# neyuru/RayTracing

Hardware: AMD Instinct MI355X
Metric: ray-steps/sec (whole node) on vert_heterogeneous, 1M rays; % HBM roofline (higher is better)
Workload: dtype f64

## Files before the change

### include/rtmi.h

```cpp
#ifndef RTMI_H
#define RTMI_H

#include <stdint.h>

#ifdef __cplusplus
extern "C" {
#endif

#define RTMI_ABI_VERSION 7

typedef enum {
    RTMI_OK = 0,
    RTMI_ERR_ARG = -1,
    RTMI_ERR_HIP = -2,
    RTMI_ERR_ALLOC = -3,
    RTMI_ERR_STATE = -4,
    RTMI_ERR_UNSUPPORTED = -5
} rtmi_status;

typedef enum { RTMI_INTERFACE = 1, RTMI_FISHEYE = 2, RTMI_VERT_HETEROGENEOUS = 3, RTMI_ANISOTROPY = 4 } rtmi_scenario;

typedef enum { RTMI_OP_MIN = 1, RTMI_OP_MAX = 11 } rtmi_method_range;

typedef enum { RTMI_F64 = 0, RTMI_F32 = 1 } rtmi_dtype;
// ... 221 lines not shown
int rtmi_kirchhoff_lsqr(rtmi_kirchhoff *k, const rtmi_lsqr_params *lp, const double *data, double *x, double *history,
                        rtmi_lsqr_stats *st);

typedef struct {
    void *s_ray, *n_ray;
    double *x, *y, *theta;
    void *n, *gx, *gy;
    double *dist_sim, *dist_real, *T;
    int32_t *istep;
    const int32_t *perm;
    int64_t R, rec_rows;
    int32_t dtype, record_stride;
} rtmi_device_view;
int rtmi_batch_view(rtmi_batch *b, rtmi_device_view *v);

#define RTMI_AUTO_SAMPLES 3
typedef struct {
    uint64_t ray_steps;
    uint64_t live_rays;
    double kernel_ms;
    uint32_t launches;
    uint32_t vgprs, sgprs, lds_bytes;
    uint32_t launch_mode_used;
    double kernel_ms_total;
    uint64_t launches_total;
    uint32_t auto_fallbacks;
    uint32_t auto_kept;
    double auto_ms[2][RTMI_AUTO_SAMPLES];
    uint32_t auto_n[2];
    uint32_t retraced;
    uint32_t retrace_overflow;
    uint64_t retraced_total;
    uint32_t dispatch_first;
    uint32_t reserved_;
} rtmi_stats;
int rtmi_batch_stats(rtmi_batch *b, rtmi_stats *s);
void rtmi_batch_destroy(rtmi_batch *b);

typedef struct rtmi_shard rtmi_shard;
typedef enum {
    RTMI_SHARD_AUTO = 0,
    RTMI_SHARD_RCCL = 1,
    RTMI_SHARD_COPY = 2
} rtmi_shard_transport;
int rtmi_shard_create(int scenario, double xi, double xs, double yi, double ys, double delta, const rtmi_params *p, int64_t R,
                      const double *x0, const double *y0, const double *theta0, const int *devices, int ndev, int transport,
                      rtmi_shard **out);
int rtmi_shard_run(rtmi_shard *s);
int rtmi_shard_reset(rtmi_shard *s);
int rtmi_shard_read_d_ray(rtmi_shard *s, double *d_ray);
int rtmi_shard_read_final(rtmi_shard *s, double *final9);
int rtmi_shard_gather_rows(rtmi_shard *s, int64_t row0, int64_t nrows, int64_t every, double **rows_dev);
int rtmi_shard_read_rows(rtmi_shard *s, int64_t row0, int64_t nrows, int64_t every, double *s_ray);
typedef struct {
    int32_t ndev, transport;
    int64_t R;
    uint64_t ray_steps, live_rays;
    double run_seconds;
    double kernel_ms_max;
    uint32_t auto_fallbacks, reserved_;
} rtmi_shard_stats;
int rtmi_shard_info(rtmi_shard *s, rtmi_shard_stats *st);
int rtmi_shard_batch(rtmi_shard *s, int i, rtmi_batch **b, int *device);
void rtmi_shard_destroy(rtmi_shard *s);

int rtmi_debug_sincos(int64_t n, const double *x, double *s, double *c);
int rtmi_debug_arctan2(int64_t n, const double *y, const double *x, double *out);
// ... 23 lines not shown
```

### raytracing_amd/_lib.py

```python
import ctypes as C
import os

_HERE = os.path.dirname(os.path.abspath(__file__))
LIB_PATH = os.environ.get("RTMI_LIB_PATH") or os.path.join(_HERE, "librtmi.so")

ABI_VERSION = 7
AUTO_SAMPLES = 3
LAUNCH_AUTO, LAUNCH_REFILL, LAUNCH_SLICED, LAUNCH_PLAIN = 0, 1, 2, 3
LAUNCH_MODES = {"auto": LAUNCH_AUTO, "refill": LAUNCH_REFILL, "sliced": LAUNCH_SLICED, "plain": LAUNCH_PLAIN, "lane": LAUNCH_PLAIN}
LAUNCH_NAMES = {LAUNCH_AUTO: "auto", LAUNCH_REFILL: "refill", LAUNCH_SLICED: "sliced", LAUNCH_PLAIN: "plain"}

_dp = C.POINTER(C.c_double)
_ip = C.POINTER(C.c_int32)


class RtmiError(RuntimeError):
    def __init__(self, code, msg):
        super().__init__(f"librtmi error {code}: {msg}")
        self.code = code


class Params(C.Structure):
    _fields_ = [("method", C.c_int32), ("dtype", C.c_int32), ("gamma", C.c_double), ("gamma_step", C.c_double),
                ("step", C.c_double), ("max_size", C.c_int32), ("record_stride", C.c_int32), ("rec_rows", C.c_int64),
                ("box", C.c_double * 4), ("launch_mode", C.c_int32), ("block_size", C.c_int32),
                ("refill_min", C.c_int32), ("exact_basis", C.c_int32),
                ("field_path", C.c_int32), ("sort_rays", C.c_int32),
                ("ext_s_ray", C.c_void_p), ("ext_n_ray", C.c_void_p), ("lazy_clear", C.c_int32), ("no_n_ray", C.c_int32), ("slice_steps", C.c_int32),
                ("reference_order", C.c_int32), ("no_retrace", C.c_int32)]


class DeviceView(C.Structure):
    _fields_ = [("s_ray", C.c_void_p), ("n_ray", C.c_void_p), ("x", C.c_void_p), ("y", C.c_void_p),
                ("theta", C.c_void_p), ("n", C.c_void_p), ("gx", C.c_void_p), ("gy", C.c_void_p),
                ("dist_sim", C.c_void_p), ("dist_real", C.c_void_p), ("T", C.c_void_p), ("istep", C.c_void_p),
                ("perm", C.c_void_p),
                ("R", C.c_int64), ("rec_rows", C.c_int64), ("dtype", C.c_int32), ("record_stride", C.c_int32)]


class Stats(C.Structure):
    _fields_ = [("ray_steps", C.c_uint64), ("live_rays", C.c_uint64), ("kernel_ms", C.c_double),
                ("launches", C.c_uint32), ("vgprs", C.c_uint32), ("sgprs", C.c_uint32), ("lds_bytes", C.c_uint32),
                ("launch_mode_used", C.c_uint32), ("kernel_ms_total", C.c_double), ("launches_total", C.c_uint64),
                ("auto_fallbacks", C.c_uint32), ("auto_kept", C.c_uint32),
                ("auto_ms", (C.c_double * AUTO_SAMPLES) * 2), ("auto_n", C.c_uint32 * 2),
                ("retraced", C.c_uint32), ("retrace_overflow", C.c_uint32), ("retraced_total", C.c_uint64),
                ("dispatch_first", C.c_uint32), ("reserved_", C.c_uint32)]


class ShardStats(C.Structure):
    _fields_ = [("ndev", C.c_int32), ("transport", C.c_int32), ("R", C.c_int64), ("ray_steps", C.c_uint64), ("live_rays", C.c_uint64),
                ("run_seconds", C.c_double), ("kernel_ms_max", C.c_double), ("auto_fallbacks", C.c_uint32), ("reserved_", C.c_uint32)]


class TwoPointParams(C.Structure):
    _fields_ = [("max_arrivals", C.c_int32), ("max_crossings", C.c_int32), ("max_iter", C.c_int32), ("reserved0", C.c_int32),
                ("tol", C.c_double), ("mem_budget", C.c_int64), ("reserved", C.c_int64 * 4)]


class TwoPointStats(C.Structure):
    _fields_ = [("iterations", C.c_int32), ("groups", C.c_int32), ("rec_rows", C.c_int64), ("overflow", C.c_uint64),
                ("fan_ms", C.c_double), ("bracket_ms", C.c_double), ("refine_ms", C.c_double), ("reserved", C.c_double * 4)]


class GridParams(C.Structure):
    _fields_ = [("gx0", C.c_double), ("gdx", C.c_double), ("nx", C.c_int64), ("gy0", C.c_double), ("gdy", C.c_double),
                ("ny", C.c_int64), ("max_gap", C.c_double), ("max_dtheta", C.c_double), ("amplitude", C.c_int32),
                ("reserved0", C.c_int32), ("reserved", C.c_int64 * 4)]


class GridStats(C.Structure):
    _fields_ = [("cells", C.c_int64), ("skipped_cells", C.c_int64), ("triangles", C.c_int64), ("folded", C.c_int64),
                ("atomics", C.c_uint64 * 3), ("pass_ms", C.c_double * 3), ("max_gap", C.c_double), ("max_dtheta", C.c_double),
                ("reserved", C.c_double * 4)]


class ArrivalParams(C.Structure):
    _fields_ = [("karr", C.c_int32), ("order", C.c_int32), ("reserved", C.c_int64 * 4)]


# ... 230 lines not shown
```

### raytracing_amd/csrc/rtmi.hip

```cpp
#include <hip/hip_runtime.h>

#include <chrono>
#include <cmath>
#include <cstdio>
#include <cstdlib>
#include <algorithm>
#include <cstring>
#include <exception>
#include <mutex>
#include <numeric>
#include <new>
#include <string>
#include <thread>
#include <utility>
#include <vector>

#include "rt_device.h"
#include "rtmi_field.h"

static thread_local std::string g_err;
static int fail(int code, const std::string& msg) {
    g_err = msg;
    return code;
}
// ... 360 lines not shown
__device__ __forceinline__ void row_store(__amdgpu_buffer_rsrc_t rs, int voff, int soff, double v) {
    __builtin_amdgcn_raw_buffer_store_b64(__builtin_bit_cast(rt_u32x2, v), rs, voff, soff, kRowStoreAux);
}
__device__ __forceinline__ void row_store(__amdgpu_buffer_rsrc_t rs, int voff, int soff, float v) {
    __builtin_amdgcn_raw_buffer_store_b32(__builtin_bit_cast(unsigned, v), rs, voff, soff, kRowStoreAux);
}
template <typename T>
__device__ __forceinline__ T* wave_uniform_ptr(T* p) {
    const unsigned long v = (unsigned long)p;
    const unsigned lo = __builtin_amdgcn_readfirstlane((unsigned)v), hi = __builtin_amdgcn_readfirstlane((unsigned)(v >> 32));
    return (T*)(((unsigned long)hi << 32) | lo);
}
template <typename T>
__device__ __forceinline__ void write_row_uniform(const BatchDev<T>& a, T* rowp, T* nrowp, int voff, const rt::Ray<T>& r) {
    int qR = (int)(a.R * (long)sizeof(T));
    asm volatile("" : "+s"(qR));
    rowp = wave_uniform_ptr(rowp);
    nrowp = wave_uniform_ptr(nrowp);
    const __amdgpu_buffer_rsrc_t rs = __builtin_amdgcn_make_buffer_rsrc(rowp, 0, 0x7fffffff, 0x00020000);
    row_store(rs, voff, 0, (T)r.x);
    row_store(rs, voff, qR, (T)r.y);
    row_store(rs, voff, 2 * qR, r.mx);
    row_store(rs, voff, 3 * qR, r.my);
    row_store(rs, voff, 4 * qR, (T)r.tt);
    row_store(rs, voff, 5 * qR, (T)r.th);
    if (nrowp) {
        const __amdgpu_buffer_rsrc_t rn = __builtin_amdgcn_make_buffer_rsrc(nrowp, 0, 0x7fffffff, 0x00020000);
        row_store(rn, voff, 0, r.nray);
    }
}

template <typename T, int METHOD, bool ISO, typename G, bool UROW, bool COH = false>
__device__ __forceinline__ void advance_loop(const BatchDev<T>& a, const rt::Consts<T>& K, G& gather, rt::Ray<T>& r, long k, int& i,
                                             bool& alive, int max_size, int nsteps, long blk) {
    const bool RECORD = a.stride != 0;
    int stride = a.stride;
    asm volatile("" : "+s"(stride));
    int until = 0;
    long row = 0;
    int rows_left = 0;
    T *rowp = nullptr, *nrowp = nullptr;
    const int voff = (int)(threadIdx.x * sizeof(T));
    if (UROW && RECORD) {
        const int i0 = __builtin_amdgcn_readfirstlane(rt::wave_max_i(alive ? i : 0));
        const int row0 = i0 / stride;
        until = stride - (i0 % stride);
        rows_left = (int)(a.rec_rows - 1 - row0 < 0x7fffffffL ? a.rec_rows - 1 - row0 : 0x7fffffffL);
        rowp = a.s_ray + (size_t)row0 * 6 * a.R + blk;
        nrowp = a.n_ray ? a.n_ray + (size_t)row0 * a.R + blk : nullptr;
    } else if (RECORD && alive) {
        until = stride - (i % stride);
        row = i / stride;
    }
    constexpr bool HOV = rt::ReportsSteep<G>::value && rt::RotatesUnit<T, METHOD>::value;
    auto one_step = [&]() -> bool {
        if (rt_ballot(alive) == 0ull) return false;
        const bool active = alive;
        ++i;
        const bool inside = rt::ray_step<T, METHOD, ISO>(a.F, K, gather, active, r, i);
        if (UROW && RECORD) {
            if (--until == 0) {
                until = stride;
                rowp += 6 * a.R;
                if (nrowp) nrowp += a.R;
                if (--rows_left >= 0 && active) write_row_uniform(a, rowp, nrowp, voff, r);
            }
        }
        if (active) {
            if (!UROW && RECORD) {
                if (--until == 0) {
                    until = stride;
                    ++row;
                    if (row < a.rec_rows) write_row(a, row, k, r);
                }
            }
// ... 2 lines not shown
                if constexpr (rt::IsExact<T, METHOD>::value) rt::ex::finish_state<rt::base_method(METHOD)>(a.F, gather, r);
                const BatchDev<T> ab = rare_batch(a);
                if constexpr (HOV) {
                    if (r.hov == INFINITY) {
                        store_ray<T, METHOD, COH, true>(ab, k, r, i, false);
                        __builtin_amdgcn_s_waitcnt(0x0F70);
                        if (!push_critical(ab, k, i)) {
                            r.hov = -INFINITY;
                            alive = !rt::outside(K, r) && (i + 1 < max_size);
                            if (alive) st_state<COH>(ab.alive + k, (unsigned char)1);
                        }
                        return true;
                    }
                }
                store_ray<T, METHOD, COH, HOV>(ab, k, r, i, false);
            }
        }
        if constexpr (rt::HasPrefetch<G>::value) gather.prefetch(a.F, alive, (T)r.x + r.ux * K.step, (T)r.y + r.uy * K.step);
        return true;
    };
    if constexpr (!rt::IsExact<T, METHOD>::value) {
        for (int it = 0; it < nsteps; it += 2) {
            if (!one_step()) break;
            if (it + 1 >= nsteps) break;
            if (!one_step()) break;
        }
    } else {
        for (int it = 0; it < nsteps; ++it)
            if (!one_step()) break;
    }
}

template <typename T, int METHOD, bool ISO, bool LDS, bool VAR, bool COH = false, bool NOFLAT = false, bool LAT = false, bool LAYER = false>
__device__ __forceinline__ bool advance_bundle(const BatchDev<T>& a, T* lds, long blk, int nsteps);

__device__ __forceinline__ unsigned xcd_grouped_block(unsigned h, unsigned nblocks) {
    constexpr unsigned G = 8;
    constexpr unsigned ROUND = 8u * G;
    if (h < nblocks / ROUND * ROUND) {
        const unsigned xcd = h & 7u, idx = h >> 3;
        return ((idx / G) * 8u + xcd) * G + idx % G;
    }
    return h;
}

constexpr bool light_method(int m) { return m == 2 || m == 6 || m == 1 || m == 7 || m == 8; }
constexpr bool heavy_method(int m) { return m == 4 || m == 5 || m >= 9; }
template <typename T> constexpr int advance_waves(int m, bool lds, int f32_waves) {
    return sizeof(T) == 4 ? f32_waves : lds ? (light_method(m) ? 4 : heavy_method(m) ? 2 : 3) : 3;
}

template <typename T, int METHOD, bool ISO, bool LDS, bool VAR, bool NOFLAT = false, bool LAYER = false>
__global__ __launch_bounds__(256, advance_waves<T>(METHOD, LDS, 4))
void k_advance(BatchDev<T> a, int nsteps) {
    __shared__ __attribute__((aligned(16))) T lds[kernel_lds_elems<T, METHOD, LDS>()];
    if (a.prio > 0) __builtin_amdgcn_s_setprio(3);
    unsigned bundle = xcd_grouped_block(blockIdx.x, gridDim.x);
    if constexpr (!NOFLAT && !LAYER && sizeof(T) == 8 && rt::rotating_method(METHOD)) {
        bundle += a.blk_rot;
        bundle = bundle >= gridDim.x ? bundle - gridDim.x : bundle;
    }
    advance_bundle<T, METHOD, ISO, LDS, VAR, false, NOFLAT, false, LAYER>(a, lds, (long)bundle * blockDim.x, nsteps);
}
template <typename T, int METHOD, bool ISO, bool NOFLAT = false, bool LAYER = false>
__global__ __launch_bounds__(256, 2) void k_advance_lat(BatchDev<T> a, int nsteps) {
    static_assert(uses_poly<T, METHOD>(), "k_advance_lat is built for the fast forms only");
    __shared__ __attribute__((aligned(16))) T lds[2];
    advance_bundle<T, METHOD, ISO, true, false, false, NOFLAT, true, LAYER>(a, lds, (long)blockIdx.x * blockDim.x, nsteps);
}
template <typename T, int METHOD, bool ISO, bool LDS, bool VAR, bool COH, bool NOFLAT, bool LAT, bool LAYER>
__device__ __forceinline__ bool advance_bundle(const BatchDev<T>& a, T* lds, long blk, int nsteps) {
    std::conditional_t<LAT, std::conditional_t<LAYER, rt::LayerLaneKept<T>, rt::PolyLaneKept<T, !NOFLAT>>,
                       typename StepGatherOf<T, METHOD, LDS, NOFLAT, LAYER>::type> gather;
    gather_init<T, LDS>(gather, lds);
    if constexpr (rt::IsExact<T, METHOD>::value && rt::ex::flat_shortcut<rt::base_method(METHOD)>()) gather_flat_bound<T>(gather, a);
    if constexpr (rt::IsExact<T, METHOD>::value) {
        if constexpr (rt::ex::inline_sincos(rt::base_method(METHOD)) || (METHOD & rt::kFastField) != 0) rt::ex::stage_sincos_tab();
    }
    const long k = blk + threadIdx.x;
    rt::Ray<T> r;
    int i = 0;
    bool alive = k < a.R && ld_state<COH>(a.alive + (k < a.R ? k : 0));
    rt::Consts<T> K = a.K;
    int max_size = a.max_size;
    if (VAR && a.vstep && k < a.R) { K.step = a.vstep[k]; K.step2h = a.vstep2h[k]; K.step2 = K.step2h * T(2); max_size = a.vmax[k]; }
    constexpr bool HOV = rt::ReportsSteep<decltype(gather)>::value && rt::RotatesUnit<T, METHOD>::value;
    if constexpr (HOV) gather.hov_limit = a.hov_limit / (float)K.step;
    if (alive) load_ray<T, METHOD, ISO, COH, HOV>(a, k, r, i);
    else idle_ray(a, r);
    __builtin_amdgcn_s_waitcnt(0x0F70);
    advance_loop<T, METHOD, ISO, decltype(gather), !VAR, COH>(a, K, gather, r, k, i, alive, max_size, nsteps, blk);
    if (alive) {
        if constexpr (rt::IsExact<T, METHOD>::value) rt::ex::finish_state<rt::base_method(METHOD)>(a.F, gather, r);
        store_ray<T, METHOD, COH, HOV>(a, k, r, i, true);
    }
    return alive;
}

__device__ __forceinline__ unsigned long long uniform_u64(unsigned long long v) {
    const unsigned lo = __builtin_amdgcn_readfirstlane((unsigned)v), hi = __builtin_amdgcn_readfirstlane((unsigned)(v >> 32));
    return ((unsigned long long)hi << 32) | lo;
}
__device__ __forceinline__ unsigned long long ld_u64(const unsigned long long* p) {
    return uniform_u64(__hip_atomic_load(p, __ATOMIC_RELAXED, __HIP_MEMORY_SCOPE_AGENT));
}
__device__ __forceinline__ unsigned long long realtime_ticks() { return __builtin_amdgcn_s_memrealtime(); }
__device__ __forceinline__ void compiler_fence() { __atomic_signal_fence(__ATOMIC_SEQ_CST); }
template <typename T, int METHOD, bool ISO, bool LDS, bool NOFLAT = false, bool LAYER = false>
__global__ __launch_bounds__(256, advance_waves<T>(METHOD, LDS, 5))
void k_advance_sliced(BatchDev<T> a, int slice, unsigned long long capacity, unsigned long long* ctl, unsigned long long timeout_ticks) {
    __shared__ __attribute__((aligned(16))) T lds[kernel_lds_elems<T, METHOD, LDS>()];
    __shared__ unsigned long long s_entry;
    const unsigned long long NB = (unsigned long long)((a.R + 255) / 256);
    unsigned long long* head = ctl;
    unsigned long long* pushed = ctl + 1;
    unsigned long long* finished = ctl + 2;
    unsigned long long* stalled = ctl + 3;
    unsigned long long* entries = ctl + 4;
    const unsigned long long kStop = ~0ull;
    const bool wave0 = __builtin_amdgcn_readfirstlane((int)(threadIdx.x >> 6)) == 0;
    const unsigned long long one = (threadIdx.x & 63) == 0 ? 1ull : 0ull;
    bool running = true;
    while (running) {
        if (wave0) {
// ... 3 lines not shown
                if (i < NB) {
                    e = i + 1ull;
                } else if (i - NB < capacity) {
                    e = ld_u64(entries + (i - NB));
                    unsigned long long f0 = ~0ull, p0 = ~0ull, t0 = realtime_ticks();
                    while (e == 0ull) {
                        const unsigned long long f = ld_u64(finished);
                        const unsigned long long p = ld_u64(pushed + (f >> 63));
                        if (f == NB + p && i >= NB + p) { e = kStop; break; }
                        const unsigned long long now = realtime_ticks();
                        if (f != f0 || p != p0) { f0 = f; p0 = p; t0 = now; }
                        else if (now - t0 > timeout_ticks) break;
                        __builtin_amdgcn_s_sleep(32);
                        e = ld_u64(entries + (i - NB));
                    }
                    if (e == 0ull) { __hip_atomic_store(stalled, 1ull, __ATOMIC_RELAXED, __HIP_MEMORY_SCOPE_AGENT); e = kStop; }
                } else {
                    __hip_atomic_store(stalled, 2ull, __ATOMIC_RELAXED, __HIP_MEMORY_SCOPE_AGENT);
                }
            }
            compiler_fence();
            s_entry = e;
        }
        __syncthreads();
        const unsigned long long e = uniform_u64(s_entry);
        __syncthreads();
        if (e == kStop) {
            running = false;
        } else {
            const long bundle = (long)((e & 0xffffffffull) - 1ull);
            const unsigned k = (unsigned)(e >> 32);
            const int nsteps = k == 0u ? 4 * slice : k == 1u ? 2 * slice : slice;
            compiler_fence();
            const bool alive = advance_bundle<T, METHOD, ISO, LDS, false, true, NOFLAT, false, LAYER>(a, lds, bundle * 256, nsteps);
            compiler_fence();
            __builtin_amdgcn_s_waitcnt(0x0F70);
            const int any = __builtin_amdgcn_readfirstlane(__syncthreads_or(alive));
            if (wave0) {
                if (any) {
                    const unsigned long long slot = uniform_u64(atomicAdd(pushed, one));
                    compiler_fence();
                    if (slot < capacity)
                        __hip_atomic_store(entries + slot, ((unsigned long long)(k + 1u) << 32) | (unsigned long long)(bundle + 1),
                                           __ATOMIC_RELAXED, __HIP_MEMORY_SCOPE_AGENT);
                    __builtin_amdgcn_s_waitcnt(0x0F70);
                }
                atomicAdd(finished, one);
            }
        }
    }
}

template <typename T, int METHOD, bool ISO, bool LDS, bool LAYER = false>
__global__ __launch_bounds__(256, sizeof(T) == 4 ? 4 : light_method(METHOD) ? 3 : 2) void k_trace_refill(BatchDev<T> a, int refill_min, int chunk) {
    __shared__ __attribute__((aligned(16))) T lds[kernel_lds_elems<T, METHOD, LDS>()];
    typename StepGatherOf<T, METHOD, LDS, false, LAYER>::type gather;
    gather_init<T, LDS>(gather, lds);
    if constexpr (rt::IsExact<T, METHOD>::value && rt::ex::flat_shortcut<rt::base_method(METHOD)>()) gather_flat_bound<T>(gather, a);
    if constexpr (rt::IsExact<T, METHOD>::value) {
        if constexpr (rt::ex::inline_sincos(rt::base_method(METHOD)) || (METHOD & rt::kFastField) != 0) rt::ex::stage_sincos_tab();
    }
    const bool RECORD = a.stride != 0;
    constexpr bool RHOV = rt::ReportsSteep<decltype(gather)>::value && rt::RotatesUnit<T, METHOD>::value;
    rt::Consts<T> K = a.K;
    if constexpr (RHOV) gather.hov_limit = a.hov_limit / (float)K.step;
    const unsigned lane = threadIdx.x & 63;
    rt::Ray<T> r;
// ... 65 lines not shown
    }
}

template <typename T> __device__ __forceinline__ int max_size_of(const BatchDev<T>& a, long k) { return a.vmax ? a.vmax[k] : a.max_size; }

template <typename T> __device__ __forceinline__ long out_index(const BatchDev<T>& a, long k) { return a.perm ? (long)a.perm[k] : k; }

template <typename T> __global__ void k_pack_d_ray(BatchDev<T> a, double* out) {
    const long k = (long)blockIdx.x * blockDim.x + threadIdx.x;
    if (k >= a.R) return;
    const long o = out_index(a, k);
    out[o] = a.acc(4)[k]; out[a.R + o] = a.acc(3)[k]; out[2 * a.R + o] = (double)a.istep[k];
}
template <typename T> __global__ void k_pack_final(BatchDev<T> a, double* out) {
    const long k = (long)blockIdx.x * blockDim.x + threadIdx.x;
    if (k >= a.R) return;
    rt::Ray<T> r;
    r.x = a.acc(0)[k]; r.y = a.acc(1)[k]; r.th = a.acc(2)[k]; r.n = a.aux(0)[k]; r.gx = a.aux(1)[k]; r.gy = a.aux(2)[k]; r.tt = a.acc(5)[k];
    if (a.rot) {
        r.ux = a.unit(0)[k]; r.uy = a.unit(1)[k];
        if (a.iso) rt::derive<T, true, true>(a.K, r); else rt::derive<T, false, true>(a.K, r);
    } else derive_rt(a, r);
    const double v[9] = {(double)r.x, (double)r.y, (double)r.th, (double)r.n, (double)r.gx, (double)r.gy,
                         (double)r.mx, (double)r.my, (double)r.tt};
    const long o = out_index(a, k);
#pragma unroll
    for (int q = 0; q < 9; q++) out[(size_t)q * a.R + o] = v[q];
}
__global__ void k_f32_to_f64(const float* in, double* out, size_t n) {
    const size_t i = (size_t)blockIdx.x * blockDim.x + threadIdx.x;
    if (i < n) out[i] = (double)in[i];
}

enum StepFlavour { kOrdinary = 0, kPerRay = 1, kFewWaves = 2 };
enum StepFlat { kFlatMap = 0, kNoFlat = 1, kLayered = 2 };
struct StepBuild {
    int dtype = RTMI_F64;
    int ki = 0;
    bool iso = false;
    bool lds = false;
    int flat = kFlatMap;
    int flavour = kOrdinary;
    int slot() const { return (iso ? 1 : 0) | (lds ? 2 : 0) | flat << 2 | flavour << 4; }
    bool operator==(const StepBuild& o) const { return dtype == o.dtype && ki == o.ki && slot() == o.slot(); }
};
struct rtmi_batch {
    const rtmi_field* field = nullptr;
    rtmi_params p{};
    int64_t R = 0;
    size_t esz = 8;
    hipStream_t stream = nullptr;
    void* state = nullptr;
    int* istep = nullptr;
    unsigned char* alive = nullptr;
    void *s_ray = nullptr, *n_ray = nullptr;
    bool own_s = false, own_n = false;
    double* launch = nullptr;
    int* perm = nullptr;
    void *vstep = nullptr, *vstep2h = nullptr;
    int* vmax = nullptr;
    unsigned long long* counters = nullptr;
    unsigned long long* h_counters = nullptr;
    std::vector<std::pair<hipEvent_t, hipEvent_t>> events;
    size_t ev_used = 0;
    size_t pass_ev_start = 0;
    double kernel_ms = 0;
    double total_kernel_ms = 0;
    uint64_t total_launches = 0;
    uint32_t launches = 0;
    int persistent_blocks = 0;
    int sliced_blocks = 0;
    unsigned long long* sliced_ctl = nullptr;
    bool dirty = false;
    bool dirty_state = false;
    bool state_rows = false;
    double auto_ms[2][RTMI_AUTO_SAMPLES] = {{0, 0, 0}, {0, 0, 0}};
    int auto_n[2] = {0, 0};
    int auto_kept = -1;
    double gold_sup[8] = {0, 0, 0, 0, 0, 0, 0, 0};
    int lat_simds = 0;
    int mode_used = RTMI_LAUNCH_PLAIN;
    const void* kfn_used = nullptr;
    uint32_t auto_fallbacks = 0;
    void* staging = nullptr;
    size_t staging_bytes = 0;
    hipGraph_t graph = nullptr;
    hipGraphExec_t graph_exec = nullptr;
    StepBuild graph_build;
    int graph_nsteps = 0, graph_count = 0, graph_block = 0;
    struct Retrace* rt = nullptr;
    bool is_retrace_sub = false;
};
static void drop_graph(rtmi_batch* b);

struct Retrace {
    rtmi_batch* sub = nullptr;
    unsigned cap = 0;
    unsigned long long* rq = nullptr;
    unsigned* host_count = nullptr;
    float* hov = nullptr;
    static constexpr int kAux = 4;
    hipStream_t aux[kAux] = {nullptr, nullptr, nullptr, nullptr};
    hipEvent_t ev_main = nullptr, ev_aux[kAux] = {nullptr, nullptr, nullptr, nullptr};
    hipStream_t masked = nullptr;
    hipEvent_t ev_in = nullptr, ev_out = nullptr;
    unsigned chunks = 0;
    unsigned launched = 0;
    unsigned scattered = 0;
    bool pending = false;
    unsigned long long* dbg = nullptr;
    unsigned overflow = 0;
    double* org = nullptr;
    int* org_istep = nullptr;
// ... 114 lines not shown
static int sliced_steps(const rtmi_batch* b) {
    const int s = b->p.slice_steps > 0 ? b->p.slice_steps : 512;
    return s < (1 << 20) ? s : (1 << 20);
}
static unsigned long long sliced_timeout_ticks(const rtmi_batch* b, int slice) {
    const double steps = std::min(4.0 * (double)slice, (double)b->p.max_size);
    const int m = b->p.method;
    const double us_per_step = (m == 5 || m >= 9) ? 200.0 : 20.0;
    const double seconds = 2.0 + steps * us_per_step * 1e-6;
    return (unsigned long long)(seconds * 1e8);
}
static bool sliced_feasible(const rtmi_batch* b) { return sliced_capacity(b, sliced_steps(b)) <= (1ull << 25); }

constexpr int kKernelMethods = 17;
constexpr int kmethod_of(int idx) {
    return idx < 11 ? idx + 1 : idx == 16 ? (7 | rt::kRefOrder | rt::kFastField) : (idx == 11 ? 1 : idx == 12 ? 2 : idx == 13 ? 6 : idx == 14 ? 7 : 8) | rt::kRefOrder;
}
static int kernel_index(int method, bool ref_order, bool fast_field) {
    if (!ref_order || rt::is_exact_method(method)) return method - 1;
    if (fast_field) return 16;
    return method == 1 ? 11 : method == 2 ? 12 : method == 6 ? 13 : method == 7 ? 14 : 15;
}
static int batch_kernel_index(const rtmi_batch* b) { return kernel_index(b->p.method, ref_order(b->p), fast_field_order(b->p)); }

static StepBuild step_build(const rtmi_batch* b) {
    StepBuild k;
    k.dtype = b->p.dtype;
    k.ki = batch_kernel_index(b);
    k.iso = b->p.gamma == 1.0 && b->p.method < 10;
    k.lds = use_lds_tile(b);
    k.flat = b->field->flat_cells != 0 || b->field->steep_cells != 0 ? kFlatMap : b->field->layered ? kLayered : kNoFlat;
    if (k.lds && k.dtype == RTMI_F64 && (b->p.method == 2 || b->p.method == 6) && !b->vstep && uniform_rows_ok(b) && !ref_order(b->p) &&
        (b->R + 63) / 64 <= (int64_t)2 * b->lat_simds)
        k.flavour = kFewWaves;
    else if (b->vstep || !uniform_rows_ok(b))
        k.flavour = kPerRay;
    return k;
}

constexpr int kSlots = 3 << 4;
template <typename T, int I, int S, int SCHED> static const void* build_kernel() {
    constexpr int M = sizeof(T) == 4 ? rt::base_method(kmethod_of(I)) : kmethod_of(I);
    constexpr bool ISO = (S & 1) && rt::base_method(M) < 10, LDS = (S & 2) != 0;
    constexpr int FLAT = (S >> 2) & 3, FLAVOUR = S >> 4;
    constexpr bool LAYER = FLAT == kLayered && sizeof(T) == 8 && uses_poly<T, M>() && !rt::IsExact<T, M>::value;
    constexpr bool NOFLAT = (FLAT == kNoFlat || FLAT == kLayered) && (LDS ? uses_poly<T, M>() : sizeof(T) == 8 && (I == 11 || I == 12 || I == 13 || I == 15));
    if constexpr (LAYER) {
        if constexpr (SCHED == RTMI_LAUNCH_SLICED) return (const void*)k_advance_sliced<T, M, ISO, LDS, true, true>;
        else if constexpr (SCHED == RTMI_LAUNCH_REFILL) return (const void*)k_trace_refill<T, M, ISO, LDS, true>;
        else if constexpr (FLAVOUR == kPerRay) return (const void*)k_advance<T, M, ISO, false, true, true, true>;
        else if constexpr (FLAVOUR == kOrdinary) return (const void*)k_advance<T, M, ISO, LDS, false, true, true>;
        else if constexpr ((M == 2 || M == 6) && LDS) return (const void*)k_advance_lat<T, M, ISO, true, true>;
        else return nullptr;
    }
    else if constexpr (SCHED == RTMI_LAUNCH_SLICED) return (const void*)k_advance_sliced<T, M, ISO, LDS, NOFLAT>;
    else if constexpr (SCHED == RTMI_LAUNCH_REFILL) return (const void*)k_trace_refill<T, M, ISO, LDS>;
    else if constexpr (FLAVOUR == kPerRay) return (const void*)k_advance<T, M, ISO, false, true>;
    else if constexpr (FLAVOUR == kOrdinary) return (const void*)k_advance<T, M, ISO, LDS, false, NOFLAT>;
    else if constexpr (sizeof(T) == 8 && (M == 2 || M == 6) && LDS) return (const void*)k_advance_lat<T, M, ISO, NOFLAT>;
    else return nullptr;
}
template <typename T, int SCHED, size_t... N> static const void* build_table(size_t n, std::index_sequence<N...>) {
    static const void* const tab[] = {build_kernel<T, (int)(N / kSlots), (int)(N % kSlots), SCHED>()...};
    return tab[n];
}
template <typename T> static const void* step_kernel_t(size_t n, int sched) {
    constexpr auto all = std::make_index_sequence<kKernelMethods * kSlots>();
    return sched == RTMI_LAUNCH_SLICED ? build_table<T, RTMI_LAUNCH_SLICED>(n, all)
         : sched == RTMI_LAUNCH_REFILL ? build_table<T, RTMI_LAUNCH_REFILL>(n, all) : build_table<T, RTMI_LAUNCH_PLAIN>(n, all);
}
static const void* step_kernel(const StepBuild& k, int sched) {
    const size_t n = (size_t)k.ki * kSlots + (size_t)k.slot();
    return by_dtype(k.dtype, [&](auto t) { return step_kernel_t<decltype(t)>(n, sched); });
}

template <typename T, typename F> static hipError_t with_step_node_t(const rtmi_batch* b, const StepBuild& k, int sched, int nsteps, F&& use) {
    BatchDev<T> a = batch_dev<T>(b);
    int refill_min = b->p.refill_min > 0 ? b->p.refill_min : 32, chunk = 16;
    unsigned long long capacity = 0, timeout = 0, *ctl = b->sliced_ctl;
    void* plain[] = {&a, &nsteps};
    void* refill[] = {&a, &refill_min, &chunk};
    void* sliced[] = {&a, &nsteps, &capacity, &ctl, &timeout};
    const long bundles = (b->R + 255) / 256;
    hipKernelNodeParams kp{};
    kp.func = const_cast<void*>(step_kernel(k, sched));
    kp.blockDim = dim3(256);
    if (sched == RTMI_LAUNCH_PLAIN) {
        const int bs = b->p.block_size > 0 ? b->p.block_size : 256;
        kp.gridDim = dim3((unsigned)((b->R + bs - 1) / bs));
        kp.blockDim = dim3(bs);
        kp.kernelParams = plain;
    } else if (sched == RTMI_LAUNCH_SLICED) {
        capacity = sliced_capacity(b, nsteps);
        timeout = sliced_timeout_ticks(b, nsteps);
        kp.gridDim = dim3((unsigned)(bundles < b->sliced_blocks ? bundles : b->sliced_blocks));
        kp.kernelParams = sliced;
    } else {
        kp.gridDim = dim3((unsigned)(bundles < b->persistent_blocks ? bundles : b->persistent_blocks));
        kp.kernelParams = refill;
    }
    return use(kp);
}
template <typename F> static hipError_t with_step_node(const rtmi_batch* b, const StepBuild& k, int sched, int nsteps, F&& use) {
    return by_dtype(k.dtype, [&](auto t) { return with_step_node_t<decltype(t)>(b, k, sched, nsteps, use); });
}

static int batch_init_state(rtmi_batch* b, bool clear_traj) {
    hipStream_t st = b->stream;
    const size_t R = (size_t)b->R;
    HIP_TRY(hipMemsetAsync(b->counters, 0, 4 * sizeof(unsigned long long), st));
    if (b->rt) { const int rcr = retrace_reset(b); if (rcr) return rcr; }
    if (clear_traj && b->s_ray) HIP_TRY(hipMemsetAsync(b->s_ray, 0, (size_t)b->p.rec_rows * 6 * R * b->esz, st));
    if (clear_traj && b->n_ray) HIP_TRY(hipMemsetAsync(b->n_ray, 0, (size_t)b->p.rec_rows * R * b->esz, st));
    b->dirty = false;
    by_dtype(b->p.dtype, [&](auto t) { hipLaunchKernelGGL(k_init<decltype(t)>, blocks(b->R), dim3(256), 0, st, batch_dev<decltype(t)>(b)); });
    HIP_TRY(hipGetLastError());
    b->kernel_ms = 0; b->launches = 0; b->pass_ev_start = b->ev_used; b->dirty_state = false;
    b->state_rows = false;
    return RTMI_OK;
}

RTMI_EXPORT void rtmi_batch_destroy(rtmi_batch* b) {
    if (!b) return;
    (void)hipStreamSynchronize(b->stream);
    (void)hipFree(b->state); (void)hipFree(b->istep); (void)hipFree(b->alive); (void)hipFree(b->launch);
    (void)hipFree(b->perm);
    (void)hipFree(b->vstep); (void)hipFree(b->vstep2h); (void)hipFree(b->vmax);
    (void)hipFree(b->counters); (void)hipFree(b->sliced_ctl); (void)hipFree(b->staging);
    if (b->h_counters) (void)hipHostFree(b->h_counters);
    if (b->own_s) (void)hipFree(b->s_ray);
    if (b->own_n) (void)hipFree(b->n_ray);
    retrace_destroy(b);
    drop_graph(b);
    for (auto& e : b->events) { (void)hipEventDestroy(e.first); (void)hipEventDestroy(e.second); }
    delete b;
}

// ... 58 lines not shown
            const double ibx = 1.0 / (16.0 * f->hx), iby = 1.0 / (16.0 * f->hy);
            auto block = [&](int k) {
                const double u = (x0[k] - f->ax) * ibx, v = (y0[k] - f->ay) * iby;
                const long bu = u >= 0 && u < 65535 ? (long)u : (u < 0 ? -1 : 65535);
                const long bv = v >= 0 && v < 65535 ? (long)v : (v < 0 ? -1 : 65535);
                return bv * 65537 + bu;
            };
            std::vector<long> key(Rz);
            for (size_t k = 0; k < Rz; k++) key[k] = block((int)k);
            std::stable_sort(perm.begin(), perm.end(), [&](int i, int j) {
                if (key[i] != key[j]) return key[i] < key[j];
                const double a = theta0[i], c = theta0[j];
                if (a == a && c == c) return a < c;
                return a == a && c != c;
            });
            sorted.resize(3 * Rz);
            for (size_t k = 0; k < Rz; k++) {
                sorted[k] = x0[perm[k]]; sorted[Rz + k] = y0[perm[k]]; sorted[2 * Rz + k] = theta0[perm[k]];
            }
            HIP_TRY(hipMalloc(&b->perm, Rz * sizeof(int)));
            HIP_TRY(hipMemcpyAsync(b->perm, perm.data(), Rz * sizeof(int), hipMemcpyHostToDevice, b->stream));
            HIP_TRY(hipMemcpyAsync(b->launch, sorted.data(), 3 * Rz * 8, hipMemcpyHostToDevice, b->stream));
            HIP_TRY(hipStreamSynchronize(b->stream));
        } else {
            HIP_TRY(hipMemcpyAsync(b->launch, x0, Rz * 8, hipMemcpyHostToDevice, b->stream));
            HIP_TRY(hipMemcpyAsync(b->launch + Rz, y0, Rz * 8, hipMemcpyHostToDevice, b->stream));
            HIP_TRY(hipMemcpyAsync(b->launch + 2 * Rz, theta0, Rz * 8, hipMemcpyHostToDevice, b->stream));
        }
        HIP_TRY(hipStreamSynchronize(b->stream));
        int dev = 0, cus = 0, per_cu = 0;
        HIP_TRY(hipGetDevice(&dev));
        HIP_TRY(hipDeviceGetAttribute(&cus, hipDeviceAttributeMultiprocessorCount, dev));
        b->lat_simds = cus * 4;
        const StepBuild k = step_build(b);
        b->kfn_used = step_kernel(k, RTMI_LAUNCH_PLAIN);
        HIP_TRY(hipOccupancyMaxActiveBlocksPerMultiprocessor(&per_cu, step_kernel(k, RTMI_LAUNCH_REFILL), 256, 0));
        b->persistent_blocks = cus * (per_cu > 0 ? per_cu : 1);
        if (b->p.launch_mode == RTMI_LAUNCH_SLICED || b->p.launch_mode == RTMI_LAUNCH_AUTO) {
            HIP_TRY(hipOccupancyMaxActiveBlocksPerMultiprocessor(&per_cu, step_kernel(k, RTMI_LAUNCH_SLICED), 256, 0));
            b->sliced_blocks = cus * (per_cu > 0 ? per_cu : 1);
            if (getenv("RTMI_DEBUG")) fprintf(stderr, "rtmi: sliced kernel: %d CUs x %d resident blocks\n", cus, per_cu);
            if (b->p.launch_mode == RTMI_LAUNCH_SLICED)
                ARG_TRY(sliced_feasible(b),
                        "rtmi_batch_create: RTMI_LAUNCH_SLICED: slice_steps too small for this batch size and max_size (queue > 256 MB)");
            const bool may_slice = b->p.launch_mode == RTMI_LAUNCH_SLICED || (sliced_feasible(b) && (R + 255) / 256 > b->sliced_blocks);
            if (may_slice)
                HIP_TRY(hipMalloc(&b->sliced_ctl, (4 + sliced_capacity(b, sliced_steps(b))) * sizeof(unsigned long long)));
        }
        if (retrace_wanted(b)) {
            const int rcr = retrace_create(b, x0, y0, theta0);
            if (rcr) return rcr;
        }
        return batch_init_state(b, true);
    };
    try {
        rc = body();
    } catch (const std::exception& e) {
        rc = fail(RTMI_ERR_ALLOC, std::string("rtmi_batch_create: ") + e.what());
    }
    if (rc) { rtmi_batch_destroy(b); return rc; }
    *out = b;
    return RTMI_OK;
}

template <typename T>
__global__ void k_set_per_ray(BatchDev<T> a, const double* step, const double* step2h, const int* ms, T* vstep, T* vstep2h, int* vmax) {
// ... 305 lines not shown
    e = hipGraphInstantiate(&b->graph_exec, b->graph, nullptr, nullptr, 0);
    if (e != hipSuccess) return e;
    b->graph_build = k; b->graph_nsteps = nsteps; b->graph_count = count; b->graph_block = bs;
    return hipSuccess;
}

RTMI_EXPORT int rtmi_step_repeat(rtmi_batch* b, int32_t nsteps, int32_t count) {
    ARG_TRY(b, "rtmi_step_repeat: null");
    ARG_TRY(nsteps > 0 && count > 0 && count <= 65536, "rtmi_step_repeat: nsteps must be > 0 and count in 1..65536");
    DEVICE_TRY(b->field, "rtmi_step_repeat");
    ARG_TRY(b->p.block_size == 0 || (b->p.block_size % 64 == 0 && b->p.block_size <= 256),
            "rtmi_step_repeat: block_size must be a multiple of 64, at most 256");
    const int bs = b->p.block_size > 0 ? b->p.block_size : 256;
    const StepBuild k = step_build(b);
    if (!b->graph_exec || !(b->graph_build == k) || b->graph_nsteps != nsteps || b->graph_count != count || b->graph_block != bs) {
        const hipError_t e = build_step_graph(b, k, nsteps, count, bs);
        if (e != hipSuccess) {
            drop_graph(b);
            (void)hipGetLastError();
            for (int i = 0; i < count; i++) { const int rc = rtmi_step(b, nsteps); if (rc) return rc; }
            return RTMI_OK;
        }
    }
    std::pair<hipEvent_t, hipEvent_t>* evp = nullptr;
    int rc0 = next_event_pair(b, &evp);
    if (rc0) return rc0;
    HIP_TRY(hipEventRecord(evp->first, b->stream));
    HIP_TRY(hipGraphLaunch(b->graph_exec, b->stream));
    if (b->rt) b->rt->pending = true;
    HIP_TRY(hipEventRecord(evp->second, b->stream));
    b->launches += (uint32_t)count; b->total_launches += (uint64_t)count;
    b->mode_used = RTMI_LAUNCH_PLAIN;
    b->kfn_used = step_kernel(k, RTMI_LAUNCH_PLAIN);
    return RTMI_OK;
}

struct OwnStream {
    rtmi_batch* b = nullptr;
    hipStream_t callers = nullptr;
    bool on = false;
    int enter(rtmi_batch* b_);
    int leave();
    ~OwnStream() { if (on) b->stream = callers; }
};

int OwnStream::enter(rtmi_batch* b_) {
    b = b_;
    callers = b->stream;
    if (!b->rt || !b->rt->masked) return RTMI_OK;
    HIP_TRY(hipEventRecord(b->rt->ev_in, callers));
    HIP_TRY(hipStreamWaitEvent(b->rt->masked, b->rt->ev_in, 0));
    b->stream = b->rt->masked;
    on = true;
    return RTMI_OK;
}
int OwnStream::leave() {
    if (!on) return RTMI_OK;
    b->stream = callers;
    on = false;
    HIP_TRY(hipEventRecord(b->rt->ev_out, b->rt->masked));
    HIP_TRY(hipStreamWaitEvent(callers, b->rt->ev_out, 0));
    return RTMI_OK;
}

static int timed_launch(rtmi_batch* b, int sched, int nsteps, bool drain, std::pair<hipEvent_t, hipEvent_t>** evp) {
    int rc = next_event_pair(b, evp);
    if (rc) return rc;
    auto* ev = *evp;
    if (sched == RTMI_LAUNCH_SLICED) HIP_TRY(hipMemsetAsync(b->sliced_ctl, 0, (4 + sliced_capacity(b, nsteps)) * sizeof(unsigned long long), b->stream));
    if (sched == RTMI_LAUNCH_REFILL) HIP_TRY(hipMemsetAsync(b->counters + 2, 0, sizeof(unsigned long long), b->stream));
    HIP_TRY(hipEventRecord(ev->first, b->stream));
    OwnStream own;
    if (drain) { const int rco = own.enter(b); if (rco) return rco; }
    (void)with_step_node(b, step_build(b), sched, nsteps, [&](const hipKernelNodeParams& kp) {
        b->kfn_used = kp.func;
        return hipLaunchKernel(kp.func, kp.gridDim, kp.blockDim, kp.kernelParams, 0, b->stream);
    });
    HIP_TRY(hipGetLastError());
    if (b->rt) {
        b->rt->pending = true;
        if (drain) { const int rcd = retrace_drain(b, true); if (rcd) return rcd; }
    }
    { const int rco = own.leave(); if (rco) return rco; }
    HIP_TRY(hipEventRecord(ev->second, b->stream));
    b->launches++; b->total_launches++;
    b->mode_used = sched;
    return RTMI_OK;
}

static int step_impl(rtmi_batch* b, int32_t nsteps, bool drain) {
    ARG_TRY(b, "rtmi_step: null");
    ARG_TRY(nsteps > 0, "rtmi_step: nsteps must be > 0");
    DEVICE_TRY(b->field, "rtmi_step");
    ARG_TRY(b->p.block_size == 0 || (b->p.block_size % 64 == 0 && b->p.block_size <= 256),
            "rtmi_step: block_size must be a multiple of 64, at most 256");
    std::pair<hipEvent_t, hipEvent_t>* evp = nullptr;
    return timed_launch(b, RTMI_LAUNCH_PLAIN, nsteps, drain, &evp);
}
RTMI_EXPORT int rtmi_step(rtmi_batch* b, int32_t nsteps) { return step_impl(b, nsteps, false); }

static int read_counters(rtmi_batch* b) {
    HIP_TRY(hipMemsetAsync(b->counters, 0, 2 * sizeof(unsigned long long), b->stream));
    hipLaunchKernelGGL(k_stats, dim3(256), dim3(256), 0, b->stream, b->istep, b->alive, (long)b->R, b->counters);
    HIP_TRY(hipGetLastError());
    HIP_TRY(hipMemcpyAsync(b->h_counters, b->counters, 2 * sizeof(unsigned long long), hipMemcpyDeviceToHost, b->stream));
    HIP_TRY(hipStreamSynchronize(b->stream));
    return RTMI_OK;
}

static bool sliced_ready(const rtmi_batch* b) { return b->sliced_ctl && !b->vstep && uniform_rows_ok(b); }

static int run_sliced(rtmi_batch* b, std::pair<hipEvent_t, hipEvent_t>** evp) {
    int rc = timed_launch(b, RTMI_LAUNCH_SLICED, sliced_steps(b), true, evp);
    if (rc) return rc;
    rc = read_counters(b);
    if (rc) return rc;
    if (b->h_counters[1] != 0) {
        unsigned long long ctl4[4] = {0, 0, 0, 0};
        HIP_TRY(hipMemcpy(ctl4, b->sliced_ctl, sizeof(ctl4), hipMemcpyDeviceToHost));
// ... 635 lines not shown

RTMI_EXPORT int rtmi_batch_view(rtmi_batch* b, rtmi_device_view* v) {
    ARG_TRY(b && v, "rtmi_batch_view: null");
    RETRACE_FLUSH(b);
    const size_t R = (size_t)b->R, e = b->esz;
    double* acc = (double*)b->state;
    char* aux = (char*)(acc + 6 * R);
    v->s_ray = b->s_ray; v->n_ray = b->n_ray;
    v->x = acc; v->y = acc + R; v->theta = acc + 2 * R; v->dist_sim = acc + 3 * R; v->dist_real = acc + 4 * R; v->T = acc + 5 * R;
    v->n = aux; v->gx = aux + R * e; v->gy = aux + 2 * R * e;
    v->perm = b->perm;
    v->istep = b->istep; v->R = b->R; v->rec_rows = b->p.rec_rows; v->dtype = b->p.dtype; v->record_stride = b->p.record_stride;
    return RTMI_OK;
}

RTMI_EXPORT int rtmi_batch_stats(rtmi_batch* b, rtmi_stats* s) {
    ARG_TRY(b && s, "rtmi_batch_stats: null");
    RETRACE_FLUSH(b);
    int rc = fold_events(b);
    if (rc) return rc;
    rc = read_counters(b);
    if (rc) return rc;
    s->ray_steps = b->h_counters[0];
    s->live_rays = b->h_counters[1];
    s->kernel_ms = b->kernel_ms;
    s->launches = b->launches;
    s->kernel_ms_total = b->total_kernel_ms;
    s->launches_total = b->total_launches;
    s->auto_fallbacks = b->auto_fallbacks;
    s->retraced = b->rt ? b->rt->scattered : 0u;
    s->retrace_overflow = b->rt ? b->rt->overflow : 0u;
    s->retraced_total = b->rt ? b->rt->total : 0ull;
    s->dispatch_first = b->rt ? b->rt->rot : 0u;
    s->reserved_ = 0;
    s->auto_kept = b->auto_kept < 0 ? 0 : b->auto_kept == 0 ? RTMI_LAUNCH_SLICED : RTMI_LAUNCH_PLAIN;
    for (int k = 0; k < 2; k++) {
        s->auto_n[k] = (uint32_t)b->auto_n[k];
        for (int i = 0; i < RTMI_AUTO_SAMPLES; i++) s->auto_ms[k][i] = i < b->auto_n[k] ? b->auto_ms[k][i] : 0.0;
    }
    hipFuncAttributes fa;
    s->vgprs = s->sgprs = s->lds_bytes = 0;
    s->launch_mode_used = (uint32_t)b->mode_used;
    if (hipFuncGetAttributes(&fa, b->kfn_used) == hipSuccess) { s->vgprs = fa.numRegs; s->lds_bytes = (uint32_t)fa.sharedSizeBytes; }
    return RTMI_OK;
}

__global__ void k_debug_sincos(long n, const double* x, double* s, double* c) {
    const long i = (long)blockIdx.x * blockDim.x + threadIdx.x;
    if (i >= n) return;
    s[i] = rt::ex::sin_(x[i]);
    c[i] = rt::ex::cos_(x[i]);
}

RTMI_EXPORT int rtmi_debug_sincos(int64_t n, const double* x, double* s, double* c) {
    ARG_TRY(x && s && c, "rtmi_debug_sincos: null");
    ARG_TRY(n >= 0, "rtmi_debug_sincos: n < 0");
    if (n == 0) return RTMI_OK;
    const char* who = "rtmi_debug_sincos";
    DevMem mem;
    double* d = nullptr;
    const size_t nb = (size_t)n * sizeof(double);
    RTMI_HIP(mem.get(&d, 3 * nb));
    RTMI_HIP(hipMemcpy(d, x, nb, hipMemcpyHostToDevice));
    hipLaunchKernelGGL(k_debug_sincos, blocks(n), dim3(256), 0, nullptr, (long)n, d, d + n, d + 2 * n);
    RTMI_HIP(hipGetLastError());
    RTMI_HIP(hipMemcpy(s, d + n, nb, hipMemcpyDeviceToHost));
    RTMI_HIP(hipMemcpy(c, d + 2 * n, nb, hipMemcpyDeviceToHost));
// ... 35 lines not shown
```

Measured before the change: 141.1 billion.

## Add paired 512-thread few-waves kernel packing two ray bundles per CU

Adds a k_advance_lat_paired kernel that launches one 512-thread workgroup per CU, with each half advancing a separate 256-ray bundle. The few-waves path selects it when there are more bundles than CUs and the field has no flat map. The bundle lane index is threaded through advance_bundle/advance_loop instead of using threadIdx.x. The aim is to place bundles evenly across CUs in the latency-bound low-ray-count regime, at the cost of launch_bounds(512,1) register limits and a new stats field.

```diff
diff --git a/include/rtmi.h b/include/rtmi.h
--- a/include/rtmi.h
+++ b/include/rtmi.h
@@ -277,7 +277,7 @@
     uint32_t retrace_overflow;
     uint64_t retraced_total;
     uint32_t dispatch_first;
-    uint32_t reserved_;
+    uint32_t paired_bundles;
 } rtmi_stats;
 int rtmi_batch_stats(rtmi_batch *b, rtmi_stats *s);
 void rtmi_batch_destroy(rtmi_batch *b);
diff --git a/raytracing_amd/_lib.py b/raytracing_amd/_lib.py
--- a/raytracing_amd/_lib.py
+++ b/raytracing_amd/_lib.py
@@ -45,7 +45,7 @@
                 ("auto_fallbacks", C.c_uint32), ("auto_kept", C.c_uint32),
                 ("auto_ms", (C.c_double * AUTO_SAMPLES) * 2), ("auto_n", C.c_uint32 * 2),
                 ("retraced", C.c_uint32), ("retrace_overflow", C.c_uint32), ("retraced_total", C.c_uint64),
-                ("dispatch_first", C.c_uint32), ("reserved_", C.c_uint32)]
+                ("dispatch_first", C.c_uint32), ("paired_bundles", C.c_uint32)]
 
 
 class ShardStats(C.Structure):
diff --git a/raytracing_amd/csrc/rtmi.hip b/raytracing_amd/csrc/rtmi.hip
--- a/raytracing_amd/csrc/rtmi.hip
+++ b/raytracing_amd/csrc/rtmi.hip
@@ -416,7 +416,7 @@
 
 template <typename T, int METHOD, bool ISO, typename G, bool UROW, bool COH = false>
 __device__ __forceinline__ void advance_loop(const BatchDev<T>& a, const rt::Consts<T>& K, G& gather, rt::Ray<T>& r, long k, int& i,
-                                             bool& alive, int max_size, int nsteps, long blk) {
+                                             bool& alive, int max_size, int nsteps, long blk, unsigned lane) {
     const bool RECORD = a.stride != 0;
     int stride = a.stride;
     asm volatile("" : "+s"(stride));
@@ -424,7 +424,7 @@
     long row = 0;
     int rows_left = 0;
     T *rowp = nullptr, *nrowp = nullptr;
-    const int voff = (int)(threadIdx.x * sizeof(T));
+    const int voff = (int)(lane * sizeof(T));
     if (UROW && RECORD) {
         const int i0 = __builtin_amdgcn_readfirstlane(rt::wave_max_i(alive ? i : 0));
         const int row0 = i0 / stride;
@@ -493,7 +493,7 @@
 }
 
 template <typename T, int METHOD, bool ISO, bool LDS, bool VAR, bool COH = false, bool NOFLAT = false, bool LAT = false, bool LAYER = false>
-__device__ __forceinline__ bool advance_bundle(const BatchDev<T>& a, T* lds, long blk, int nsteps);
+__device__ __forceinline__ bool advance_bundle(const BatchDev<T>& a, T* lds, long blk, unsigned lane, int nsteps);
 
 __device__ __forceinline__ unsigned xcd_grouped_block(unsigned h, unsigned nblocks) {
     constexpr unsigned G = 8;
@@ -521,16 +521,25 @@
         bundle += a.blk_rot;
         bundle = bundle >= gridDim.x ? bundle - gridDim.x : bundle;
     }
-    advance_bundle<T, METHOD, ISO, LDS, VAR, false, NOFLAT, false, LAYER>(a, lds, (long)bundle * blockDim.x, nsteps);
+    advance_bundle<T, METHOD, ISO, LDS, VAR, false, NOFLAT, false, LAYER>(a, lds, (long)bundle * blockDim.x, threadIdx.x, nsteps);
 }
 template <typename T, int METHOD, bool ISO, bool NOFLAT = false, bool LAYER = false>
 __global__ __launch_bounds__(256, 2) void k_advance_lat(BatchDev<T> a, int nsteps) {
     static_assert(uses_poly<T, METHOD>(), "k_advance_lat is built for the fast forms only");
     __shared__ __attribute__((aligned(16))) T lds[2];
-    advance_bundle<T, METHOD, ISO, true, false, false, NOFLAT, true, LAYER>(a, lds, (long)blockIdx.x * blockDim.x, nsteps);
+    advance_bundle<T, METHOD, ISO, true, false, false, NOFLAT, true, LAYER>(a, lds, (long)blockIdx.x * blockDim.x, threadIdx.x, nsteps);
+}
+template <typename T, int METHOD, bool ISO, bool NOFLAT = false, bool LAYER = false>
+__global__ __launch_bounds__(512, 1) void k_advance_lat_paired(BatchDev<T> a, int nsteps) {
+    static_assert(uses_poly<T, METHOD>(), "k_advance_lat_paired is built for the fast forms only");
+    __shared__ __attribute__((aligned(16))) T lds[2];
+    const unsigned half = (unsigned)__builtin_amdgcn_readfirstlane((int)(threadIdx.x >> 8));
+    const long blk = ((long)blockIdx.x + (long)half * gridDim.x) * 256;
+    if (blk >= a.R) return;
+    advance_bundle<T, METHOD, ISO, true, false, false, NOFLAT, true, LAYER>(a, lds, blk, threadIdx.x & 255u, nsteps);
 }
 template <typename T, int METHOD, bool ISO, bool LDS, bool VAR, bool COH, bool NOFLAT, bool LAT, bool LAYER>
-__device__ __forceinline__ bool advance_bundle(const BatchDev<T>& a, T* lds, long blk, int nsteps) {
+__device__ __forceinline__ bool advance_bundle(const BatchDev<T>& a, T* lds, long blk, unsigned lane, int nsteps) {
     std::conditional_t<LAT, std::conditional_t<LAYER, rt::LayerLaneKept<T>, rt::PolyLaneKept<T, !NOFLAT>>,
                        typename StepGatherOf<T, METHOD, LDS, NOFLAT, LAYER>::type> gather;
     gather_init<T, LDS>(gather, lds);
@@ -538,7 +547,7 @@
     if constexpr (rt::IsExact<T, METHOD>::value) {
         if constexpr (rt::ex::inline_sincos(rt::base_method(METHOD)) || (METHOD & rt::kFastField) != 0) rt::ex::stage_sincos_tab();
     }
-    const long k = blk + threadIdx.x;
+    const long k = blk + lane;
     rt::Ray<T> r;
     int i = 0;
     bool alive = k < a.R && ld_state<COH>(a.alive + (k < a.R ? k : 0));
@@ -550,7 +559,7 @@
     if (alive) load_ray<T, METHOD, ISO, COH, HOV>(a, k, r, i);
     else idle_ray(a, r);
     __builtin_amdgcn_s_waitcnt(0x0F70);
-    advance_loop<T, METHOD, ISO, decltype(gather), !VAR, COH>(a, K, gather, r, k, i, alive, max_size, nsteps, blk);
+    advance_loop<T, METHOD, ISO, decltype(gather), !VAR, COH>(a, K, gather, r, k, i, alive, max_size, nsteps, blk, lane);
     if (alive) {
         if constexpr (rt::IsExact<T, METHOD>::value) rt::ex::finish_state<rt::base_method(METHOD)>(a.F, gather, r);
         store_ray<T, METHOD, COH, HOV>(a, k, r, i, true);
@@ -620,7 +629,7 @@
             const unsigned k = (unsigned)(e >> 32);
             const int nsteps = k == 0u ? 4 * slice : k == 1u ? 2 * slice : slice;
             compiler_fence();
-            const bool alive = advance_bundle<T, METHOD, ISO, LDS, false, true, NOFLAT, false, LAYER>(a, lds, bundle * 256, nsteps);
+            const bool alive = advance_bundle<T, METHOD, ISO, LDS, false, true, NOFLAT, false, LAYER>(a, lds, bundle * 256, threadIdx.x, nsteps);
             compiler_fence();
             __builtin_amdgcn_s_waitcnt(0x0F70);
             const int any = __builtin_amdgcn_readfirstlane(__syncthreads_or(alive));
@@ -752,7 +761,7 @@
     if (i < n) out[i] = (double)in[i];
 }
 
-enum StepFlavour { kOrdinary = 0, kPerRay = 1, kFewWaves = 2 };
+enum StepFlavour { kOrdinary = 0, kPerRay = 1, kFewWaves = 2, kFewWavesPaired = 3 };
 enum StepFlat { kFlatMap = 0, kNoFlat = 1, kLayered = 2 };
 struct StepBuild {
     int dtype = RTMI_F64;
@@ -799,6 +808,8 @@
     int auto_kept = -1;
     double gold_sup[8] = {0, 0, 0, 0, 0, 0, 0, 0};
     int lat_simds = 0;
+    int pair_groups = 0;
+    uint32_t paired = 0;
     int mode_used = RTMI_LAUNCH_PLAIN;
     const void* kfn_used = nullptr;
     uint32_t auto_fallbacks = 0;
@@ -979,13 +990,14 @@
     k.flat = b->field->flat_cells != 0 || b->field->steep_cells != 0 ? kFlatMap : b->field->layered ? kLayered : kNoFlat;
     if (k.lds && k.dtype == RTMI_F64 && (b->p.method == 2 || b->p.method == 6) && !b->vstep && uniform_rows_ok(b) && !ref_order(b->p) &&
         (b->R + 63) / 64 <= (int64_t)2 * b->lat_simds)
-        k.flavour = kFewWaves;
+        k.flavour = b->pair_groups > 0 && (b->R + 255) / 256 > b->pair_groups && k.flat != kFlatMap &&
+                    (b->p.block_size == 0 || b->p.block_size == 256) ? kFewWavesPaired : kFewWaves;
     else if (b->vstep || !uniform_rows_ok(b))
         k.flavour = kPerRay;
     return k;
 }
 
-constexpr int kSlots = 3 << 4;
+constexpr int kSlots = 4 << 4;
 template <typename T, int I, int S, int SCHED> static const void* build_kernel() {
     constexpr int M = sizeof(T) == 4 ? rt::base_method(kmethod_of(I)) : kmethod_of(I);
     constexpr bool ISO = (S & 1) && rt::base_method(M) < 10, LDS = (S & 2) != 0;
@@ -997,14 +1009,16 @@
         else if constexpr (SCHED == RTMI_LAUNCH_REFILL) return (const void*)k_trace_refill<T, M, ISO, LDS, true>;
         else if constexpr (FLAVOUR == kPerRay) return (const void*)k_advance<T, M, ISO, false, true, true, true>;
         else if constexpr (FLAVOUR == kOrdinary) return (const void*)k_advance<T, M, ISO, LDS, false, true, true>;
-        else if constexpr ((M == 2 || M == 6) && LDS) return (const void*)k_advance_lat<T, M, ISO, true, true>;
+        else if constexpr (FLAVOUR == kFewWaves && (M == 2 || M == 6) && LDS) return (const void*)k_advance_lat<T, M, ISO, true, true>;
+        else if constexpr (FLAVOUR == kFewWavesPaired && (M == 2 || M == 6) && LDS) return (const void*)k_advance_lat_paired<T, M, ISO, true, true>;
         else return nullptr;
     }
     else if constexpr (SCHED == RTMI_LAUNCH_SLICED) return (const void*)k_advance_sliced<T, M, ISO, LDS, NOFLAT>;
     else if constexpr (SCHED == RTMI_LAUNCH_REFILL) return (const void*)k_trace_refill<T, M, ISO, LDS>;
     else if constexpr (FLAVOUR == kPerRay) return (const void*)k_advance<T, M, ISO, false, true>;
     else if constexpr (FLAVOUR == kOrdinary) return (const void*)k_advance<T, M, ISO, LDS, false, NOFLAT>;
-    else if constexpr (sizeof(T) == 8 && (M == 2 || M == 6) && LDS) return (const void*)k_advance_lat<T, M, ISO, NOFLAT>;
+    else if constexpr (FLAVOUR == kFewWaves && sizeof(T) == 8 && (M == 2 || M == 6) && LDS) return (const void*)k_advance_lat<T, M, ISO, NOFLAT>;
+    else if constexpr (FLAVOUR == kFewWavesPaired && sizeof(T) == 8 && (M == 2 || M == 6) && LDS && NOFLAT) return (const void*)k_advance_lat_paired<T, M, ISO, true>;
     else return nullptr;
 }
 template <typename T, int SCHED, size_t... N> static const void* build_table(size_t n, std::index_sequence<N...>) {
@@ -1036,6 +1050,10 @@
         const int bs = b->p.block_size > 0 ? b->p.block_size : 256;
         kp.gridDim = dim3((unsigned)((b->R + bs - 1) / bs));
         kp.blockDim = dim3(bs);
+        if (k.flavour == kFewWavesPaired) {
+            kp.gridDim = dim3((unsigned)b->pair_groups);
+            kp.blockDim = dim3(512);
+        }
         kp.kernelParams = plain;
     } else if (sched == RTMI_LAUNCH_SLICED) {
         capacity = sliced_capacity(b, nsteps);
@@ -1050,6 +1068,10 @@
 }
 template <typename F> static hipError_t with_step_node(const rtmi_batch* b, const StepBuild& k, int sched, int nsteps, F&& use) {
     return by_dtype(k.dtype, [&](auto t) { return with_step_node_t<decltype(t)>(b, k, sched, nsteps, use); });
+}
+
+static uint32_t paired_bundles(const rtmi_batch* b, const StepBuild& k, int sched) {
+    return sched == RTMI_LAUNCH_PLAIN && k.flavour == kFewWavesPaired ? (uint32_t)((b->R + 255) / 256 - b->pair_groups) : 0u;
 }
 
 static int batch_init_state(rtmi_batch* b, bool clear_traj) {
@@ -1174,6 +1196,15 @@
         HIP_TRY(hipGetDevice(&dev));
         HIP_TRY(hipDeviceGetAttribute(&cus, hipDeviceAttributeMultiprocessorCount, dev));
         b->lat_simds = cus * 4;
+        {
+            StepBuild kpair = step_build(b);
+            kpair.flavour = kFewWavesPaired;
+            const void* fpair = step_kernel(kpair, RTMI_LAUNCH_PLAIN);
+            if (fpair) {
+                HIP_TRY(hipOccupancyMaxActiveBlocksPerMultiprocessor(&per_cu, fpair, 512, 0));
+                if (per_cu == 1) b->pair_groups = cus;
+            }
+        }
         const StepBuild k = step_build(b);
         b->kfn_used = step_kernel(k, RTMI_LAUNCH_PLAIN);
         HIP_TRY(hipOccupancyMaxActiveBlocksPerMultiprocessor(&per_cu, step_kernel(k, RTMI_LAUNCH_REFILL), 256, 0));
@@ -1545,6 +1576,7 @@
     b->launches += (uint32_t)count; b->total_launches += (uint64_t)count;
     b->mode_used = RTMI_LAUNCH_PLAIN;
     b->kfn_used = step_kernel(k, RTMI_LAUNCH_PLAIN);
+    b->paired = paired_bundles(b, k, RTMI_LAUNCH_PLAIN);
     return RTMI_OK;
 }
 
@@ -1585,7 +1617,8 @@
     HIP_TRY(hipEventRecord(ev->first, b->stream));
     OwnStream own;
     if (drain) { const int rco = own.enter(b); if (rco) return rco; }
-    (void)with_step_node(b, step_build(b), sched, nsteps, [&](const hipKernelNodeParams& kp) {
+    const StepBuild k = step_build(b);
+    (void)with_step_node(b, k, sched, nsteps, [&](const hipKernelNodeParams& kp) {
         b->kfn_used = kp.func;
         return hipLaunchKernel(kp.func, kp.gridDim, kp.blockDim, kp.kernelParams, 0, b->stream);
     });
@@ -1598,6 +1631,7 @@
     HIP_TRY(hipEventRecord(ev->second, b->stream));
     b->launches++; b->total_launches++;
     b->mode_used = sched;
+    b->paired = paired_bundles(b, k, sched);
     return RTMI_OK;
 }
 
@@ -2299,7 +2333,7 @@
     s->retrace_overflow = b->rt ? b->rt->overflow : 0u;
     s->retraced_total = b->rt ? b->rt->total : 0ull;
     s->dispatch_first = b->rt ? b->rt->rot : 0u;
-    s->reserved_ = 0;
+    s->paired_bundles = b->paired;
     s->auto_kept = b->auto_kept < 0 ? 0 : b->auto_kept == 0 ? RTMI_LAUNCH_SLICED : RTMI_LAUNCH_PLAIN;
     for (int k = 0; k < 2; k++) {
         s->auto_n[k] = (uint32_t)b->auto_n[k];
```

Measured after the change: 136.7 billion. 0.968x the previous value.
